# openfheorg/openfhe-boolean-circuit-evaluator

Measured on NVIDIA B200. Metric: bootstrapped gates/sec (STD128_OPT GINX), higher is better.
Workload: dtype u32

## Files before the change

openfhe-boolean-circuit-evaluator_b200/csrc/kernels.cu:

```cuda
#include "device.cuh"
#include <type_traits>
#include <cuda_runtime.h>
#include <cstdlib>

namespace bfhe {

constexpr int SOL_LAT_WIDE = 0x05, SOL_LAT_NARROW = 0x0a;

__device__ __forceinline__ u32 f_phys(u32 u) { return (u & ~31u) | ((u ^ (u >> 5)) & 31u); }
template <int E> struct Lay {
  static constexpr int C = E / 4;
  __device__ __forceinline__ static int swz(int tp) { return E == 32 ? (tp & 7) : ((tp >> 1) & 3); }
  __device__ __forceinline__ static int chunk_off(int tp, int c) { return E * tp + 4 * (c ^ swz(tp)); }
  __device__ __forceinline__ static int elem_off(int k, int lane) {
    if (E == 32) return 32 * k + 4 * ((lane >> 2) ^ (k & 7)) + (lane & 3);
    int j = lane & 15;
    return 16 * (2 * k + (lane >> 4)) + 4 * ((j >> 2) ^ (k & 3)) + (j & 3);
  }
};
template <int E> __device__ __forceinline__ void row_load(const u32 *buf, u32 (&x)[E], int lane) {
#pragma unroll
  for (int c = 0; c < E / 4; c++) {
    uint4 v = *reinterpret_cast<const uint4 *>(buf + Lay<E>::chunk_off(lane, c));
    x[4 * c] = v.x; x[4 * c + 1] = v.y; x[4 * c + 2] = v.z; x[4 * c + 3] = v.w;
// ... 78 lines not shown
        x[a] = RED ? lazy_reduce(S, Q) : S;
      }
    }
    if constexpr (!LAST) GsRun<E, 2 * T, OUTB, UNI, MAXLAST>::run(x, utw, utws, Q, tab, tabs, lane);
  }
};
__host__ __device__ constexpr int gs_out_bound(int E, int B0, int MAXLAST) {
  int B = B0;
  for (int T = 1; T < E; T *= 2) {
    const int NB = 2 * B;
    const bool last = 2 * T >= E;
    B = (last ? NB > MAXLAST : NB > 16) ? 2 : NB;
  }
  return B;
}

struct TwTabs {
  const u32 *fw, *fws, *iw, *iws;
};

template <int LOGN, bool PRE = false, int SOLW = 0, int SOLN = 0>
__device__ __forceinline__ void ntt_forward(u32 (&x)[(1 << LOGN) / 32], u32 *buf, const DevConst &P, const TwTabs &tt, int lane,
                                            const u32 *pre = nullptr) {
  constexpr int E = (1 << LOGN) / 32;
  const u32 Q = P.Q, Q2 = P.Q2;
  ct_pass<E, true, SOLW, PRE>(x, P.tw, P.tws, Q, Q2, nullptr, nullptr, 0, pre);
  if constexpr (LOGN & 1) {
    const bool up = lane & 16;
#pragma unroll
    for (int k = 0; k < E; k++) {
      u32 v = up ? mul_shoup(x[k], P.tw[16 + k], P.tws[16 + k], Q) : x[k];
      u32 o = __shfl_xor_sync(0xffffffffu, v, 16);
      x[k] = up ? (o - v + Q2) : (v + o);
    }
  }
  __syncwarp();
  col_store<E>(buf, x, lane);
  __syncwarp();
  row_load<E>(buf, x, lane);
  ct_pass<E, false, SOLN>(x, P.tw, P.tws, Q, Q2, tt.fw, tt.fws, lane);
}

template <int LOGN, int B0>
__device__ __forceinline__ void ntt_inverse(u32 (&x)[(1 << LOGN) / 32], u32 *buf, const DevConst &P, const TwTabs &tt, int lane) {
  constexpr int E = (1 << LOGN) / 32;
  const u32 Q = P.Q;
  constexpr int ML = (LOGN & 1) ? 8 : 16;
  GsRun<E, 1, B0, false, ML>::run(x, P.itw, P.itws, Q, tt.iw, tt.iws, lane);
  constexpr int B1 = gs_out_bound(E, B0, ML);
  __syncwarp();
  row_store<E>(buf, x, lane);
  __syncwarp();
  col_load<E>(buf, x, lane);
  if constexpr (LOGN & 1) {
    static_assert(B1 <= 8, "bound");
    const bool up = lane & 16;
    const u32 off = B1 * Q;
#pragma unroll
    for (int k = 0; k < E; k++) {
      u32 o = __shfl_xor_sync(0xffffffffu, x[k], 16);
      u32 D = o - x[k] + off;
      x[k] = up ? mul_shoup(D, P.itw[16 + k], P.itws[16 + k], Q) : (x[k] + o);
    }
    constexpr int B2 = 2 * B1;
    GsRun<E, 1, B2, true, 32>::run(x, P.itw, P.itws, Q);
  } else {
    GsRun<E, 1, B1, true, 32>::run(x, P.itw, P.itws, Q);
  }
#pragma unroll
  for (int k = 0; k < E; k++) x[k] = csub(lazy_reduce(x[k], Q), Q);
}

__device__ __forceinline__ u32 brev(u32 x, int bits) { return __brev(x) >> (32 - bits); }
template <int DG, int LOGBG> constexpr u32 digit_offset() {
  u32 off = 0;
  for (int l = 0; l < DG; l++) off += (1u << (LOGBG - 1)) << (LOGBG * l);
  return off;
}

template <int LOGN, int DG, int LOGBG, int G, bool AP> struct BrCfg {
  static constexpr int N = 1 << LOGN, E = N / 32, C = E / 4, ROWS = 2 * DG;
  static constexpr int W = 2 * G, THREADS = 32 * W;
  static constexpr int NPAD = AP ? 1024 : 512;
  static constexpr size_t dct_words = (size_t)G * ROWS * N;
  static constexpr bool LUT = (LOGBG == 7 && LOGN == 10);
  static constexpr size_t lut_words = LUT ? (size_t)32 << LOGBG : 0;
  static constexpr bool FOLD = LUT && !AP;
  static constexpr size_t smem_bytes = (dct_words + 4 * N + (AP ? 0 : 2 * N) + lut_words) * 4 + (size_t)G * NPAD * 2;
};

template <int LOGN, int DG, int LOGBG, int G, bool AP>
__global__ void __launch_bounds__(64 * G, 1)
blind_rotate_kernel(const __grid_constant__ DevConst P, const DevGate *__restrict__ gates, int count,
                    const u32 *__restrict__ bk, const u32 *__restrict__ g_twl, const u32 *__restrict__ g_psiM,
                    u32 *__restrict__ ext, u32 *__restrict__ acc_dbg) {
  using Cfg = BrCfg<LOGN, DG, LOGBG, G, AP>;
  constexpr int N = Cfg::N, E = Cfg::E, C = Cfg::C, ROWS = Cfg::ROWS, W = Cfg::W, NPAD = Cfg::NPAD;
  constexpr u32 DIGIT_OFF = digit_offset<DG, LOGBG>();
  constexpr bool FOLD = Cfg::FOLD;
  static_assert(!FOLD || (DIGIT_OFF >= (SOLINAS_Q + 1) / 2 && (u64)DIGIT_OFF + (SOLINAS_Q - 3) / 2 < (1ull << (LOGBG * DG))),
                "the digits do not cover the centred accumulator: the top digit cannot be folded into the key");
  constexpr int ND = FOLD ? DG - 1 : DG;
  extern __shared__ __align__(128) unsigned char smem_raw[];
  u32 *dct = reinterpret_cast<u32 *>(smem_raw);
  u32 *s_tw = dct + Cfg::dct_words;
  u32 *s_psiM = s_tw + 4 * N;
  u32 *s_lut = s_psiM + (AP ? 0 : 2 * N);
  u16 *s_idx = reinterpret_cast<u16 *>(s_lut + Cfg::lut_words);

  const int tid = threadIdx.x, lane = tid & 31, warp = tid >> 5;
  const int g = warp >> 1, c = warp & 1;
  if constexpr (Cfg::LUT) {
    for (int i = tid; i < (int)Cfg::lut_words; i += Cfg::THREADS) {
      const u32 d = (u32)i >> 5;
      s_lut[i] = (u32)(((u64)P.tw[1] * ((d + P.Q - (1u << (LOGBG - 1))) % P.Q)) % P.Q);
    }
  }
  const int gate0 = blockIdx.x * G;
  const int gcount = min(G, count - gate0);
  const u32 Q = P.Q, q = P.q, n = P.n;

  for (int i = tid; i < 4 * N; i += Cfg::THREADS) s_tw[i] = g_twl[i];
  if (!AP)
    for (int u = tid; u < N; u += Cfg::THREADS) s_psiM[f_phys((u32)u)] = (g_psiM[2 * u] + (P.Q - P.oneM)) % P.Q;
  const TwTabs tt{s_tw, s_tw + N, s_tw + 2 * N, s_tw + 3 * N};

  __shared__ u32 s_b[G];
  for (int gg = 0; gg < gcount; gg++) {
    const DevGate dg = gates[gate0 + gg];
    const u32 gate = dg.op & 0xff;
    for (u32 i = tid; i <= n; i += Cfg::THREADS) {
      u32 x = dg.in0[i];
      if (dg.op & OP_NEG0) x = (i == n) ? (q / 4 + q - x) % q : (q - x) % q;
      u32 v;
      if (gate == OP_BOOTSTRAP) {
        v = (i == n) ? (x + q / 4) % q : x;
      } else {
        u32 y = dg.in1[i];
        if (dg.op & OP_NEG1) y = (i == n) ? (q / 4 + q - y) % q : (q - y) % q;
        v = (gate == OP_XOR_FAST || gate == OP_XNOR_FAST) ? (2 * (x + q - y)) % q : (x + y) % q;
      }
      if (i == n) s_b[gg] = v;
      else {
        u32 aneg = (q - v) % q;
        if (!AP) s_idx[gg * NPAD + i] = (u16)(aneg * P.factor);
        else {
          u32 a = aneg;
          for (u32 k = 0; k < P.dR; k++, a /= P.baseR) s_idx[gg * NPAD + i * P.dR + k] = (u16)(a % P.baseR);
        }
      }
    }
  }
  __syncthreads();

  const bool gvalid = g < gcount;
  u32 acc[E];
#pragma unroll
  for (int k = 0; k < E; k++) acc[k] = 0;
  if (gvalid && c == 1) {
    const u32 gate = gates[gate0 + g].op & 0xff;
    const u32 q1 = P.gate_const[gate == OP_BOOTSTRAP ? OP_AND : gate], q2 = (q1 + q / 2) % q;
    const u32 b = s_b[g], Q8 = P.Q8, Q8n = Q - P.Q8;
#pragma unroll
    for (int k = 0; k < E; k++) {
      const u32 idx = lane + 32 * k;
      if (idx % P.factor == 0) {
        const u32 t = (b + q - idx / P.factor) % q;
        const bool in = (q1 < q2) ? (t >= q1 && t < q2) : !(t >= q2 && t < q1);
        acc[k] = in ? Q8n : Q8;
      }
    }
  }
  if (FOLD && gvalid) {
    u32 x[E];
#pragma unroll
    for (int k = 0; k < E; k++) x[k] = acc[k];
    u32 *abuf = dct + ((size_t)g * ROWS + 2 * (DG - 1) + c) * N;
    ntt_forward<LOGN>(x, abuf, P, tt, lane);
#pragma unroll
    for (int k = 0; k < E; k++) x[k] = mul_shoup(x[k], P.ninv, P.ninvs, Q);
    row_store<E>(abuf, x, lane);
  }

  const int nsteps = AP ? n * P.dR : n;
  bool pending = false;
  u32 *mybuf = dct + ((size_t)g * ROWS + c) * N;

  constexpr int GS = (W >= C) ? (W / C) : 1;
  const u32 eA = 2 * brev(lane, 5) + 1;
  constexpr bool KEY_HOIST = !AP;

#ifdef BFHE_PHASE_TIMING
  long long tpt[5] = {0, 0, 0, 0, 0}, tq0 = clock64(), tq1;
#define PT_T(i) do { tq1 = clock64(); tpt[i] += tq1 - tq0; tq0 = tq1; } while (0)
#else
#define PT_T(i)
#endif
  for (int step = 0; step < nsteps; step++) {
    uint4 kr[2][ROWS][2];
#define BFHE_GX_LOAD(qc)                                     \
  do {                                                                                                                 \
    const u32 *kb_ = bk + (size_t)step * (2 * ROWS * 2) * N + ((qc) * 32 + lane) * 4;                                  \
    _Pragma("unroll") for (int s = 0; s < 2; s++)                                                                      \
      _Pragma("unroll") for (int r = 0; r < ROWS; r++)                                                                 \
        _Pragma("unroll") for (int cc = 0; cc < 2; cc++)                                                               \
          kr[s][r][cc] = __ldg(reinterpret_cast<const uint4 *>(kb_ + (size_t)((s * ROWS + r) * 2 + cc) * N));           \
  } while (0)
    constexpr int JN = (G + GS - 1) / GS;
    auto ap_key = [&](int gg, int qc) -> const u32 * {
      const u32 a0 = gg < gcount ? s_idx[gg * NPAD + step] : 0u;
      const u32 i = step / P.dR, k = step % P.dR;
      return bk + (((size_t)i * (P.baseR - 1) + (a0 ? a0 - 1 : 0u)) * P.dR + k) * (ROWS * 2) * N + (qc * 32 + lane) * 4;
    };
#define BFHE_AP_LOAD(buf, kb)                                                                                          \
  do {                                                                                                                 \
    const u32 *kb_ = (kb);                                                                                             \
    _Pragma("unroll") for (int r = 0; r < ROWS; r++)                                                                   \
      _Pragma("unroll") for (int cc = 0; cc < 2; cc++)                                                                 \
        kr[buf][r][cc] = __ldg(reinterpret_cast<const uint4 *>(kb_ + (size_t)(r * 2 + cc) * N));                        \
  } while (0)

    bool active = gvalid;
    if (AP && gvalid) active = s_idx[g * NPAD + step] != 0;
    if (active) {
      if (pending) {
        u32 x[E];
        row_load<E>(mybuf, x, lane);
        ntt_inverse<LOGN, AP ? 8 : 4>(x, mybuf, P, tt, lane);
#pragma unroll
        for (int k = 0; k < E; k++) acc[k] = AP ? x[k] : csub(acc[k] + x[k], Q);
      }
      u32 dp[E];
#pragma unroll
      for (int k = 0; k < E; k++) dp[k] = ((acc[k] < (Q >> 1)) ? acc[k] : acc[k] - Q) + DIGIT_OFF;
#pragma unroll
      for (int l = 0; l < ND; l++) {
        u32 x[E], pre[Cfg::LUT ? E / 2 : 1];
#pragma unroll
        for (int k = 0; k < E; k++) {
          const u32 dgt = (dp[k] >> (LOGBG * l)) & ((1u << LOGBG) - 1);
          if (Cfg::LUT && k >= E / 2) { pre[Cfg::LUT ? k - E / 2 : 0] = s_lut[(dgt << 5) + lane]; x[k] = 0; }
          else x[k] = dgt + (Q - (1u << (LOGBG - 1)));
        }
        u32 *buf = dct + ((size_t)g * ROWS + c + 2 * l) * N;
        if (KEY_HOIST && l == ND - 1 && warp < C * GS) BFHE_GX_LOAD(warp % C);
        ntt_forward<LOGN, Cfg::LUT>(x, buf, P, tt, lane, pre);
        row_store<E>(buf, x, lane);
      }
    } else if (KEY_HOIST && warp < C * GS) {
      BFHE_GX_LOAD(warp % C);
    }
    pending = pending || active;
    PT_T(0);
    if (AP && warp < C * GS) {
      BFHE_AP_LOAD(0, ap_key(warp / C, warp % C));
      if (JN > 1) BFHE_AP_LOAD(1, ap_key(warp / C + GS, warp % C));
    }
    __syncthreads();
    PT_T(1);

    for (int item = warp; item < C * GS; item += W) {
      const int qc = item % C, gs0 = item / C;
      if (!AP && item != warp) BFHE_GX_LOAD(qc);
      u32 eB[4];
#pragma unroll
      for (int r = 0; r < 4; r++) eB[r] = 2 * ((brev(r, 2) << (LOGN - 2)) | (brev(qc, LOGN - 7) << 5));

      if (AP && item != warp) {
        BFHE_AP_LOAD(0, ap_key(gs0, qc));
        if (JN > 1) BFHE_AP_LOAD(1, ap_key(gs0 + GS, qc));
      }
#pragma unroll
      for (int j = 0; j < JN; j++) {
        const int gg = gs0 + j * GS;
        const bool ap_active = AP && gg < gcount && s_idx[(gg < gcount ? gg : 0) * NPAD + step] != 0;
        if (gg >= gcount || (AP && !ap_active)) {
          if (AP && j + 2 < JN) { if ((j & 1) == 0) BFHE_AP_LOAD(0, ap_key(gs0 + (j + 2) * GS, qc)); else BFHE_AP_LOAD(1, ap_key(gs0 + (j + 2) * GS, qc)); }
          continue;
        }
        u32 fp[4], fn[4];
        if (!AP) {
          const u32 m = s_idx[gg * NPAD + step];
#pragma unroll
          for (int r = 0; r < 4; r++) {
            const u32 u = ((m * (eA + eB[r])) >> 1) & (N - 1);
            fp[r] = s_psiM[f_phys(u)];
            fn[r] = s_psiM[f_phys((0u - u) & (N - 1))];
          }
        }
        u32 *gd = dct + (size_t)gg * ROWS * N + Lay<E>::chunk_off(lane, qc);
        uint4 dv[ROWS];
#pragma unroll
        for (int r = 0; r < ROWS; r++) dv[r] = *reinterpret_cast<const uint4 *>(gd + (size_t)r * N);
#pragma unroll
        for (int cc = 0; cc < 2; cc++) {
          u32 out[4];
#pragma unroll
          for (int sl = 0; sl < 4; sl++) {
            u64 sp = 0, sn = 0;
#pragma unroll
            for (int r = 0; r < ROWS; r++) {
              const u32 dval = sl == 0 ? dv[r].x : sl == 1 ? dv[r].y : sl == 2 ? dv[r].z : dv[r].w;
              const uint4 kp = kr[AP ? (j & 1) : 0][r][cc];
              sp += (u64)dval * (sl == 0 ? kp.x : sl == 1 ? kp.y : sl == 2 ? kp.z : kp.w);
              if (!AP) {
                const uint4 kn = kr[AP ? 0 : 1][r][cc];
                sn += (u64)dval * (sl == 0 ? kn.x : sl == 1 ? kn.y : sl == 2 ? kn.z : kn.w);
              }
            }
            const u32 pp = redc(sp, Q, P.qinv_neg);
            if (AP) out[sl] = pp;
            else {
              const u32 pn = redc(sn, Q, P.qinv_neg);
              out[sl] = redc((u64)pp * fp[sl] + (u64)pn * fn[sl], Q, P.qinv_neg);
            }
          }
          *reinterpret_cast<uint4 *>(gd + (size_t)cc * N) = make_uint4(out[0], out[1], out[2], out[3]);
          if constexpr (FOLD) {
            const uint4 a = dv[ROWS - 2 + cc];
            *reinterpret_cast<uint4 *>(gd + (size_t)(ROWS - 2 + cc) * N) =
                make_uint4(lazy_reduce(a.x + out[0], Q), lazy_reduce(a.y + out[1], Q), lazy_reduce(a.z + out[2], Q), lazy_reduce(a.w + out[3], Q));
          }
        }
        if (AP && j + 2 < JN) {
          if ((j & 1) == 0) BFHE_AP_LOAD(0, ap_key(gs0 + (j + 2) * GS, qc)); else BFHE_AP_LOAD(1, ap_key(gs0 + (j + 2) * GS, qc));
        }
      }
    }
    PT_T(2);
    __syncthreads();
    PT_T(3);
  }

  if (gvalid) {
    if (pending) {
      u32 x[E];
      row_load<E>(mybuf, x, lane);
      ntt_inverse<LOGN, AP ? 8 : 4>(x, mybuf, P, tt, lane);
#pragma unroll
      for (int k = 0; k < E; k++) acc[k] = AP ? x[k] : csub(acc[k] + x[k], Q);
    }
    const size_t gi = (size_t)gate0 + g;
    if (acc_dbg) {
#pragma unroll
      for (int k = 0; k < E; k++) acc_dbg[(gi * 2 + c) * N + lane + 32 * k] = acc[k];
    }
    u32 *e = ext + gi * (N + 4);
    const u64 qKS = P.qKS;
    if (c == 0) {
#pragma unroll
      for (int k = 0; k < E; k++) {
        const u32 j = lane + 32 * k;
        const u32 v = (j == 0) ? acc[k] : (acc[k] == 0 ? 0 : Q - acc[k]);
        const u32 pos = (j == 0) ? 0 : N - j;
        e[pos] = (qKS == Q) ? v : (u32)(((2 * (u64)v * qKS + Q) / (2 * (u64)Q)) % qKS);
      }
    } else if (lane == 0) {
      const u32 v = csub(acc[0] + P.Q8, Q);
      e[N] = (qKS == Q) ? v : (u32)(((2 * (u64)v * qKS + Q) / (2 * (u64)Q)) % qKS);
    }
#ifdef BFHE_PHASE_TIMING
    if (acc_dbg && lane == 0)
      for (int i = 0; i < 5; i++) acc_dbg[(gi * 2 + c) * N + 32 + i] = (u32)(tpt[i] / 1000);
#endif
  }
}



template <int T, int B> struct Gs8Stage {
  static constexpr bool RED = (2 * B > 16);
  static constexpr int OUTB = RED ? 2 : 2 * B;
  __device__ __forceinline__ static void run(u32 (&x)[8], const u32 (&w)[8], const u32 (&ws)[8], u32 Q) {
    static_assert(B <= 16, "bound");
#pragma unroll
    for (int i = 0; i < 4; i++) {
      const int gi = i / T, a = gi * 2 * T + (i % T), b = a + T, p = 4 / T + gi;
      const u32 S = x[a] + x[b], D = x[a] - x[b] + B * Q;
      x[b] = mul_shoup(D, w[p], ws[p], Q);
      x[a] = RED ? lazy_reduce(S, Q) : S;
    }
  }
};
template <int B0> __device__ __forceinline__ void ntt_inverse_quad8(u32 (&x)[8], u32 *buf, const DevConst &P, const u32 *nat, const u32 *nats, int T,
                                                                   int bar_id) {
  const u32 Q = P.Q;
  u32 w[8], ws[8];
  auto run3 = [&](auto BC) {
    constexpr int B = decltype(BC)::value;
    using S1 = Gs8Stage<1, B>; using S2 = Gs8Stage<2, S1::OUTB>; using S3 = Gs8Stage<4, S2::OUTB>;
    S1::run(x, w, ws, Q); S2::run(x, w, ws, Q); S3::run(x, w, ws, Q);
  };
  constexpr int B1 = Gs8Stage<4, Gs8Stage<2, Gs8Stage<1, B0>::OUTB>::OUTB>::OUTB;
  constexpr int B2 = Gs8Stage<4, Gs8Stage<2, Gs8Stage<1, B1>::OUTB>::OUTB>::OUTB;
  constexpr int B3 = Gs8Stage<4, Gs8Stage<2, Gs8Stage<1, B2>::OUTB>::OUTB>::OUTB;
  {
    const int tp = T >> 2, c0 = 2 * (T & 3), T3 = T >> 1, hb = T & 1;
    u32 *p0 = buf + Lay<32>::chunk_off(tp, c0), *p1 = buf + Lay<32>::chunk_off(tp, c0 + 1);
    const uint4 a0 = *reinterpret_cast<const uint4 *>(p0), a1 = *reinterpret_cast<const uint4 *>(p1);
    x[0] = a0.x; x[1] = a0.y; x[2] = a0.z; x[3] = a0.w; x[4] = a1.x; x[5] = a1.y; x[6] = a1.z; x[7] = a1.w;
    const uint4 t4 = *reinterpret_cast<const uint4 *>(nat + 512 + 256 * hb + 4 * T3), t4s = *reinterpret_cast<const uint4 *>(nats + 512 + 256 * hb + 4 * T3);
    const uint2 t2 = *reinterpret_cast<const uint2 *>(nat + 256 + 2 * T), t2s = *reinterpret_cast<const uint2 *>(nats + 256 + 2 * T);
    w[4] = t4.x; w[5] = t4.y; w[6] = t4.z; w[7] = t4.w; ws[4] = t4s.x; ws[5] = t4s.y; ws[6] = t4s.z; ws[7] = t4s.w;
    w[2] = t2.x; w[3] = t2.y; ws[2] = t2s.x; ws[3] = t2s.y;
    w[1] = nat[128 + T]; ws[1] = nats[128 + T];
    run3(std::integral_constant<int, B0>{});
    *reinterpret_cast<uint4 *>(p0) = make_uint4(x[0], x[1], x[2], x[3]);
    *reinterpret_cast<uint4 *>(p1) = make_uint4(x[4], x[5], x[6], x[7]);
  }
  bar_sync(bar_id, 128);
  {
    const int u = T >> 3, v = T & 7;
    const int b = 64 * u + 8 * (u & 3) + 4 * (v >> 2) + (v & 3);
    const uint4 t4 = *reinterpret_cast<const uint4 *>(nat + 64 + 4 * u), t4s = *reinterpret_cast<const uint4 *>(nats + 64 + 4 * u);
    const uint2 t2 = *reinterpret_cast<const uint2 *>(nat + 32 + 2 * u), t2s = *reinterpret_cast<const uint2 *>(nats + 32 + 2 * u);
    w[4] = t4.x; w[5] = t4.y; w[6] = t4.z; w[7] = t4.w; ws[4] = t4s.x; ws[5] = t4s.y; ws[6] = t4s.z; ws[7] = t4s.w;
    w[2] = t2.x; w[3] = t2.y; ws[2] = t2s.x; ws[3] = t2s.y;
    w[1] = nat[16 + u]; ws[1] = nats[16 + u];
#pragma unroll
    for (int r = 0; r < 8; r++) x[r] = buf[b ^ (32 * (r >> 2) + 8 * (r & 3) + 4 * (r >> 2))];
    run3(std::integral_constant<int, B1>{});
#pragma unroll
    for (int r = 0; r < 8; r++) buf[b ^ (32 * (r >> 2) + 8 * (r & 3) + 4 * (r >> 2))] = x[r];
  }
// ... 288 lines not shown
    } else if (lane == 0) {
      e[N] = modswitch(csub(acc[0] + P.Q8, Q));
    }
  }
#ifdef BFHE_PHASE_TIMING
  if (acc_dbg && lane == 0 && (QUAD ? (q4 == 0) : (warp < 2)))
    for (int i = 0; i < 5; i++) acc_dbg[(gi * 2 + (QUAD ? qc : warp)) * N + 32 + i] = (u32)(tph[i] / 1000);
#endif
}

template <int LOGN, int DG, int LOGBG, bool AP>
static int launch_lat_inst(const DevConst &P, const DevGate *d_gates, int count, const u32 *d_bk, const u32 *d_twl,
                           const u32 *d_psiM, u32 *d_ext, u32 *d_acc, cudaStream_t st, LaunchInfo *info) {
  using Cfg = LatCfg<LOGN, DG, LOGBG, AP>;
  auto kern = blind_rotate_lat_kernel<LOGN, DG, LOGBG, AP>;
  static bool attr_done[64];
  if (int rc = once_per_device(attr_done, [&] { return cudaFuncSetAttribute(kern, cudaFuncAttributeMaxDynamicSharedMemorySize, (int)Cfg::smem_bytes); }))
    return rc;
  if (count <= 0) return 0;
  if (info) { info->gates_per_cta = 1; info->ctas = count; info->smem_bytes = Cfg::smem_bytes; }
  kern<<<count, Cfg::THREADS, Cfg::smem_bytes, st>>>(P, d_gates, count, d_bk, d_twl, d_psiM, d_ext, d_acc);
  return (int)cudaGetLastError();
}

template <int LOGN, int DG, int LOGBG, int G, bool AP>
static int launch_br_inst(const DevConst &P, const DevGate *d_gates, int count, const u32 *d_bk, const u32 *d_twl,
                          const u32 *d_psiM, u32 *d_ext, u32 *d_acc, cudaStream_t st, LaunchInfo *info) {
  using Cfg = BrCfg<LOGN, DG, LOGBG, G, AP>;
  auto kern = blind_rotate_kernel<LOGN, DG, LOGBG, G, AP>;
  static bool attr_done[64];
  if (int rc = once_per_device(attr_done, [&] { return cudaFuncSetAttribute(kern, cudaFuncAttributeMaxDynamicSharedMemorySize, (int)Cfg::smem_bytes); }))
    return rc;
  if (count <= 0) return 0;
  const int ctas = (count + G - 1) / G;
  if (info) { info->gates_per_cta = G; info->ctas = ctas; info->smem_bytes = Cfg::smem_bytes; }
  kern<<<ctas, Cfg::THREADS, Cfg::smem_bytes, st>>>(P, d_gates, count, d_bk, d_twl, d_psiM, d_ext, d_acc);
  return (int)cudaGetLastError();
}

template <int LOGN, int DG, int LOGBG, bool AP>
static int launch_br_g(int G, const DevConst &P, const DevGate *d_gates, int count, const u32 *d_bk, const u32 *d_twl,
                       const u32 *d_psiM, u32 *d_ext, u32 *d_acc, cudaStream_t st, LaunchInfo *info) {
  switch (G) {
  case 1: return launch_br_inst<LOGN, DG, LOGBG, 1, AP>(P, d_gates, count, d_bk, d_twl, d_psiM, d_ext, d_acc, st, info);
  case 2: return launch_br_inst<LOGN, DG, LOGBG, 2, AP>(P, d_gates, count, d_bk, d_twl, d_psiM, d_ext, d_acc, st, info);
  default: return launch_br_inst<LOGN, DG, LOGBG, 4, AP>(P, d_gates, count, d_bk, d_twl, d_psiM, d_ext, d_acc, st, info);
  }
}

template <int LOGN, int DG, int LOGBG> static int br_attrs() {
  DevConst P{};
  int rc = 0;
  for (int G : {1, 2, 4}) {
    rc |= launch_br_g<LOGN, DG, LOGBG, false>(G, P, nullptr, 0, nullptr, nullptr, nullptr, nullptr, nullptr, 0, nullptr);
    rc |= launch_br_g<LOGN, DG, LOGBG, true>(G, P, nullptr, 0, nullptr, nullptr, nullptr, nullptr, nullptr, 0, nullptr);
  }
  rc |= launch_lat_inst<LOGN, DG, LOGBG, false>(P, nullptr, 0, nullptr, nullptr, nullptr, nullptr, nullptr, 0, nullptr);
  rc |= launch_lat_inst<LOGN, DG, LOGBG, true>(P, nullptr, 0, nullptr, nullptr, nullptr, nullptr, nullptr, 0, nullptr);
  return rc;
}
int blind_rotate_set_attrs() {
  int rc = br_attrs<10, 4, 7>();
  rc |= br_attrs<9, 3, 9>();
  rc |= v2_set_attrs();
  rc |= clx_set_attrs();
  return rc;
}

int launch_blind_rotate(const DevConst &P, int method_ap, const DevGate *d_gates, int count, const u32 *d_bk, const u32 *d_twl,
                        const u32 *d_psiM, u32 *d_ext, u32 *d_acc_dbg, int force_g, void *stream, LaunchInfo *info, const V2Bufs *v2) {
  if (count <= 0) return 0;
  cudaStream_t st = (cudaStream_t)stream;
  const bool have_cl2 = v2 && v2->d_bk4 && v2->d_tw2 && v2->d_F && v2_supported(P, method_ap);
  const bool have_clx = v2 && v2->d_bkx && v2->d_twx && (method_ap || v2->d_F) && clx_supported(P, method_ap);
  if (force_g == 128) return have_clx ? launch_blind_rotate_clx(P, method_ap, d_gates, count, *v2, d_ext, d_acc_dbg, stream, info) : (int)cudaErrorInvalidValue;
  if (force_g == 32) return have_cl2 ? launch_blind_rotate_cl2(P, d_gates, count, *v2, d_ext, d_acc_dbg, stream, info) : (int)cudaErrorInvalidValue;
  if (force_g != 0 && force_g != 1 && force_g != 2 && force_g != 4 && force_g != 8) return (int)cudaErrorInvalidValue;
  int dev = 0, sms = 148;
  cudaGetDevice(&dev);
  cudaDeviceGetAttribute(&sms, cudaDevAttrMultiProcessorCount, dev);
  if (force_g == 0 && have_clx && count <= clx_fast_gates()) return launch_blind_rotate_clx(P, method_ap, d_gates, count, *v2, d_ext, d_acc_dbg, stream, info);
  if (force_g == 0 && have_cl2 && count <= cl2_max_gates()) return launch_blind_rotate_cl2(P, d_gates, count, *v2, d_ext, d_acc_dbg, stream, info);
  const long lat_cost = (long)((count + sms - 1) / sms) * 222;
  const long thr_cost = (long)((count + 4 * sms - 1) / (4 * sms)) * 597;
  const bool lat = force_g == 8 || (force_g == 0 && lat_cost <= thr_cost);
  if (lat) {
    if (P.N == 1024 && P.dG == 4 && P.logBG == 7)
      return method_ap ? launch_lat_inst<10, 4, 7, true>(P, d_gates, count, d_bk, d_twl, d_psiM, d_ext, d_acc_dbg, st, info)
                       : launch_lat_inst<10, 4, 7, false>(P, d_gates, count, d_bk, d_twl, d_psiM, d_ext, d_acc_dbg, st, info);
    if (P.N == 512 && P.dG == 3 && P.logBG == 9)
      return method_ap ? launch_lat_inst<9, 3, 9, true>(P, d_gates, count, d_bk, d_twl, d_psiM, d_ext, d_acc_dbg, st, info)
                       : launch_lat_inst<9, 3, 9, false>(P, d_gates, count, d_bk, d_twl, d_psiM, d_ext, d_acc_dbg, st, info);
    return (int)cudaErrorInvalidValue;
  }
  int G = force_g > 0 ? force_g : 4;
  if (P.N == 1024 && P.dG == 4 && P.logBG == 7) {
    if (method_ap) return launch_br_g<10, 4, 7, true>(G, P, d_gates, count, d_bk, d_twl, d_psiM, d_ext, d_acc_dbg, st, info);
    static_assert(BrCfg<10, 4, 7, 4, false>::FOLD, "the GINX throughput kernel of this shape reads the folded key");
    if (!v2 || !v2->d_bkf) return (int)cudaErrorInvalidValue;
    return launch_br_g<10, 4, 7, false>(G, P, d_gates, count, v2->d_bkf, d_twl, d_psiM, d_ext, d_acc_dbg, st, info);
  }
  if (P.N == 512 && P.dG == 3 && P.logBG == 9) {
    return method_ap ? launch_br_g<9, 3, 9, true>(G, P, d_gates, count, d_bk, d_twl, d_psiM, d_ext, d_acc_dbg, st, info)
                     : launch_br_g<9, 3, 9, false>(G, P, d_gates, count, d_bk, d_twl, d_psiM, d_ext, d_acc_dbg, st, info);
  }
  return (int)cudaErrorInvalidValue;
}

__device__ __forceinline__ void peer_store(const PeerX &px, const u32 *out, int k, u32 v) {
  if (px.slabs == nullptr) return;
  const size_t off = (size_t)(out - px.local_base) + (size_t)k;
  for (u32 r = 0; r < px.world; r++)
    if (r != px.rank) px.slabs[r][off] = v;
}
__device__ __forceinline__ void st_release_sys(u32 *p, u32 v) { asm volatile("st.release.sys.global.u32 [%0], %1;" ::"l"(p), "r"(v) : "memory"); }
__device__ __forceinline__ u32 ld_acquire_sys(const u32 *p) {
  u32 v;
  asm volatile("ld.acquire.sys.global.u32 %0, [%1];" : "=r"(v) : "l"(p) : "memory");
  return v;
}
__device__ __forceinline__ void peer_publish(const PeerX &px, u32 total) {
  if (px.slabs == nullptr) return;
  __threadfence_system();
  __syncthreads();
  if (threadIdx.x == 0) {
    const u32 done = atomicAdd(px.counter, 1u) + 1u;
    if (done == total) {
      atomicExch(px.counter, 0u);
      __threadfence_system();
      const u32 v = *px.epoch * px.per_epoch + px.index + 1u;
      for (u32 r = 0; r < px.world; r++)
        if (r != px.rank) st_release_sys(px.flags[r] + px.rank, v);
    }
  }
}
__global__ void peer_epoch_bump_kernel(u32 *epoch) { *epoch += 1; }
__global__ void peer_wait_kernel(const u32 *flags, const u32 *epoch, u32 world, u32 rank, int index, u32 per_epoch, u32 *err, long long timeout_cycles) {
  const u32 r = threadIdx.x;
  if (r >= world || r == rank) return;
  const u32 target = *epoch * per_epoch + (u32)(index + 1);
  const long long t0 = clock64();
  while ((int)(ld_acquire_sys(flags + r) - target) < 0) {
    if (clock64() - t0 > timeout_cycles) { atomicExch(err, 1u + r); break; }
    __nanosleep(200);
  }
}
__global__ void peer_signal_kernel(const PeerX px) {
  const u32 r = threadIdx.x;
  if (r >= px.world || r == px.rank) return;
  __threadfence_system();
  st_release_sys(px.flags[r] + px.rank, *px.epoch * px.per_epoch + px.index + 1u);
}
int launch_peer_epoch_bump(u32 *epoch, void *stream) {
  peer_epoch_bump_kernel<<<1, 1, 0, (cudaStream_t)stream>>>(epoch);
  return (int)cudaGetLastError();
}
int launch_peer_wait(const u32 *local_flags, const u32 *epoch, u32 world, u32 rank, int index, u32 per_epoch, u32 *err, void *stream) {
  if (world > 32) return (int)cudaErrorInvalidValue;
  static const long long cycles = [] {
    const char *e = std::getenv("BFHE_EXCHANGE_TIMEOUT_S");
    const double sec = e && std::atof(e) > 0 ? std::atof(e) : 30.0;
    return (long long)(sec * 2.0e9);
  }();
  peer_wait_kernel<<<1, 32, 0, (cudaStream_t)stream>>>(local_flags, epoch, world, rank, index, per_epoch, err, cycles);
  return (int)cudaGetLastError();
}
int launch_peer_signal(const PeerX &px, void *stream) {
// ... 332 lines not shown
```

openfhe-boolean-circuit-evaluator_b200/host/circuit.cpp:

```cpp
#include "../csrc/engine.hpp"
#include "netlist.hpp"
#include <algorithm>
#include <chrono>
#include <cstdio>
#include <cstdlib>
#include <cstring>
#include <dlfcn.h>
#include <queue>

using namespace bfhe;

namespace {

struct Id128 { char b[128]; };
struct NcclApi {
  void *h = nullptr;
  int (*GetUniqueId)(void *) = nullptr;
  int (*CommInitRank)(void **, int, Id128, int) = nullptr;
  int (*AllGather)(const void *, void *, size_t, int, void *, cudaStream_t) = nullptr;
  int (*Broadcast)(const void *, void *, size_t, int, int, void *, cudaStream_t) = nullptr;
  int (*CommDestroy)(void *) = nullptr;
  const char *(*GetErrorString)(int) = nullptr;
};
NcclApi g_nccl;
bool load_nccl() {
  if (g_nccl.h) return true;
  void *h = dlopen("libnccl.so.2", RTLD_NOW | RTLD_GLOBAL);
  if (!h) h = dlopen("libnccl.so", RTLD_NOW | RTLD_GLOBAL);
  if (!h) { set_error(std::string("cannot load NCCL: ") + dlerror()); return false; }
  g_nccl.GetUniqueId = (decltype(g_nccl.GetUniqueId))dlsym(h, "ncclGetUniqueId");
  g_nccl.CommInitRank = (decltype(g_nccl.CommInitRank))dlsym(h, "ncclCommInitRank");
  g_nccl.AllGather = (decltype(g_nccl.AllGather))dlsym(h, "ncclAllGather");
  g_nccl.Broadcast = (decltype(g_nccl.Broadcast))dlsym(h, "ncclBroadcast");
  g_nccl.CommDestroy = (decltype(g_nccl.CommDestroy))dlsym(h, "ncclCommDestroy");
  g_nccl.GetErrorString = (decltype(g_nccl.GetErrorString))dlsym(h, "ncclGetErrorString");
  if (!g_nccl.GetUniqueId || !g_nccl.CommInitRank || !g_nccl.AllGather || !g_nccl.Broadcast || !g_nccl.CommDestroy) {
    set_error("NCCL symbols missing");
    return false;
  }
  g_nccl.h = h;
  return true;
}
constexpr int NCCL_UINT32 = 3, NCCL_FLOAT32 = 7;

struct NotOp { uint32_t in_row, out_row, copy; };
struct Level {
  std::vector<bfhe_gate> gates;
  uint32_t first_row = 0;
  std::vector<NotOp> nots;
  bool sharded = true;
};
struct FormCosts {
  double cl4 = 1.05, cl2 = 1.55, lat = 2.36, thr = 6.1, exchange = exchange_default();
  bool measured = false;
  static double exchange_default() { const char *m = std::getenv("BFHE_EXCHANGE"); return m && std::strcmp(m, "nccl") == 0 ? 0.05 : 0.015; }
};
inline bool is_single(GateKind k) {
  return k == GateKind::AND || k == GateKind::OR || k == GateKind::NAND || k == GateKind::NOR || k == GateKind::XOR_FAST || k == GateKind::XNOR_FAST;
}
inline bool is_boot(GateKind k) { return is_single(k) || k == GateKind::XOR; }
inline uint32_t op_of(GateKind k) {
  switch (k) {
  case GateKind::AND: return BFHE_AND;
  case GateKind::OR: return BFHE_OR;
  case GateKind::NAND: return BFHE_NAND;
  case GateKind::NOR: return BFHE_NOR;
  case GateKind::XOR_FAST: return BFHE_XOR_FAST;
  default: return BFHE_XNOR_FAST;
  }
}

}

struct bfhe_circuit {
  bfhe_ctx *ctx = nullptr;
  Netlist nl;
  Netlist nl_file;
  bool loaded = false;
  bool plaintext = false, encrypted = false, verify = false;
  bool planned_verify = false;
  int rank = 0, world = 1;
  void *comm = nullptr;

  bool planned = false;
  std::vector<uint32_t> topo;
  std::vector<uint32_t> wire_row;
  std::vector<uint8_t> wire_neg;
  std::vector<uint32_t> wire_level;
  std::vector<Level> levels;
  std::vector<uint32_t> level_rpr;
  uint32_t total_rows = 0, fresh_base = 0, n_in = 0;
  std::vector<uint32_t> in_wire_of_bit;
  std::vector<uint32_t> out_wire;
  uint32_t n_bootstraps = 0, max_width = 0, asap_levels = 0;
  uint32_t wave_cap = 0;
  int wave_cap_req = -1;
  int shard_min_req = -1;
  FormCosts costs;
  uint32_t n_dff = 0, state_base = 0, dff_tmp_base = 0, dff_fresh_base = 0;
  std::vector<uint32_t> dff_gate;
  std::vector<NotOp> dff_ops;
  std::vector<uint8_t> plain_state;
  bool state_init_pending = true;
  uint64_t clocks = 0;

  uint32_t *slab = nullptr;
  DevGate *d_desc = nullptr;
  std::vector<size_t> desc_off;
  std::vector<uint32_t> my_count;
  const u32 **d_not_in = nullptr;
  u32 **d_not_out = nullptr;
  std::vector<size_t> not_off;
  u32 *d_ext = nullptr;
  size_t ext_cap = 0;
  bool dev_ready = false;
  cudaGraphExec_t graph = nullptr;
  bool use_graph = true;
  bool peer_ok = false;
  std::vector<void *> peer_slab_map, peer_flag_map;
  u32 **d_peer_slabs = nullptr, **d_peer_flags = nullptr;
  u32 *x_flags = nullptr, *x_counter = nullptr, *x_epoch = nullptr, *x_err = nullptr;
  uint32_t x_per_epoch = 1;
  std::vector<int> shard_index;

  std::vector<uint8_t> in_bits_set, plain_wire;
  bool has_input = false, done = false;
  double device_ms = 0, host_ms = 0;
  uint64_t verify_mismatches = 0, verify_checked = 0;
};

static void free_device(bfhe_circuit *c) {
  if (c->ctx && c->ctx->device >= 0) {
    cudaSetDevice(c->ctx->device);
    cudaStreamSynchronize(c->ctx->stream);
    if (c->graph) cudaGraphExecDestroy(c->graph);
    for (void *m : c->peer_slab_map) if (m) cudaIpcCloseMemHandle(m);
// ... 1093 lines not shown
```

Measured before the change: 97800.

## Keep blind-rotate accumulator in NTT domain in shared memory across steps

The throughput blind-rotate kernel now keeps the accumulator transformed (A_hat rows in shared memory) for every configuration. The external product adds into A_hat directly, and each step recovers the coefficient form with one inverse NTT of A_hat. Before, it inverted the product and added it to a register accumulator. This removes the pending-accumulate bookkeeping and register-resident acc across steps. For the non-fold cases it costs two extra shared-memory rows per gate and an extra NTT at setup. The host cost-model constants for the throughput path are lowered to match.

Result: faster. 101,900 (median of 6 runs) (+4.2%).

```diff
diff --git a/openfhe-boolean-circuit-evaluator_b200/csrc/kernels.cu b/openfhe-boolean-circuit-evaluator_b200/csrc/kernels.cu
--- a/openfhe-boolean-circuit-evaluator_b200/csrc/kernels.cu
+++ b/openfhe-boolean-circuit-evaluator_b200/csrc/kernels.cu
@@ -184,11 +184,14 @@
   static constexpr int N = 1 << LOGN, E = N / 32, C = E / 4, ROWS = 2 * DG;
   static constexpr int W = 2 * G, THREADS = 32 * W;
   static constexpr int NPAD = AP ? 1024 : 512;
-  static constexpr size_t dct_words = (size_t)G * ROWS * N;
   static constexpr bool LUT = (LOGBG == 7 && LOGN == 10);
   static constexpr size_t lut_words = LUT ? (size_t)32 << LOGBG : 0;
   static constexpr bool FOLD = LUT && !AP;
+  static constexpr int DROWS = (FOLD || AP) ? ROWS : ROWS + 2;
+  static constexpr int AROW = AP ? 0 : DROWS - 2;
+  static constexpr size_t dct_words = (size_t)G * DROWS * N;
   static constexpr size_t smem_bytes = (dct_words + 4 * N + (AP ? 0 : 2 * N) + lut_words) * 4 + (size_t)G * NPAD * 2;
+  static_assert(smem_bytes <= 227 * 1024, "more dynamic shared memory than a block may have");
 };
 
 template <int LOGN, int DG, int LOGBG, int G, bool AP>
@@ -203,6 +206,9 @@
   static_assert(!FOLD || (DIGIT_OFF >= (SOLINAS_Q + 1) / 2 && (u64)DIGIT_OFF + (SOLINAS_Q - 3) / 2 < (1ull << (LOGBG * DG))),
                 "the digits do not cover the centred accumulator: the top digit cannot be folded into the key");
   constexpr int ND = FOLD ? DG - 1 : DG;
+  constexpr int DROWS = Cfg::DROWS, AROW = Cfg::AROW;
+  static_assert(AP || AROW == 2 * ND, "GINX: the A_hat rows follow the digit rows");
+  constexpr int AB = AP ? 8 : 2;
   extern __shared__ __align__(128) unsigned char smem_raw[];
   u32 *dct = reinterpret_cast<u32 *>(smem_raw);
   u32 *s_tw = dct + Cfg::dct_words;
@@ -256,37 +262,33 @@
   __syncthreads();
 
   const bool gvalid = g < gcount;
-  u32 acc[E];
-#pragma unroll
-  for (int k = 0; k < E; k++) acc[k] = 0;
-  if (gvalid && c == 1) {
-    const u32 gate = gates[gate0 + g].op & 0xff;
-    const u32 q1 = P.gate_const[gate == OP_BOOTSTRAP ? OP_AND : gate], q2 = (q1 + q / 2) % q;
-    const u32 b = s_b[g], Q8 = P.Q8, Q8n = Q - P.Q8;
-#pragma unroll
-    for (int k = 0; k < E; k++) {
-      const u32 idx = lane + 32 * k;
-      if (idx % P.factor == 0) {
-        const u32 t = (b + q - idx / P.factor) % q;
-        const bool in = (q1 < q2) ? (t >= q1 && t < q2) : !(t >= q2 && t < q1);
-        acc[k] = in ? Q8n : Q8;
-      }
-    }
-  }
-  if (FOLD && gvalid) {
-    u32 x[E];
-#pragma unroll
-    for (int k = 0; k < E; k++) x[k] = acc[k];
-    u32 *abuf = dct + ((size_t)g * ROWS + 2 * (DG - 1) + c) * N;
-    ntt_forward<LOGN>(x, abuf, P, tt, lane);
-#pragma unroll
-    for (int k = 0; k < E; k++) x[k] = mul_shoup(x[k], P.ninv, P.ninvs, Q);
-    row_store<E>(abuf, x, lane);
+  u32 *ahat = dct + ((size_t)g * DROWS + AROW + c) * N;
+  u32 *dbuf = dct + ((size_t)g * DROWS + c) * N;
+  if (gvalid) {
+    u32 acc[E];
+#pragma unroll
+    for (int k = 0; k < E; k++) acc[k] = 0;
+    if (c == 1) {
+      const u32 gate = gates[gate0 + g].op & 0xff;
+      const u32 q1 = P.gate_const[gate == OP_BOOTSTRAP ? OP_AND : gate], q2 = (q1 + q / 2) % q;
+      const u32 b = s_b[g], Q8 = P.Q8, Q8n = Q - P.Q8;
+#pragma unroll
+      for (int k = 0; k < E; k++) {
+        const u32 idx = lane + 32 * k;
+        if (idx % P.factor == 0) {
+          const u32 t = (b + q - idx / P.factor) % q;
+          const bool in = (q1 < q2) ? (t >= q1 && t < q2) : !(t >= q2 && t < q1);
+          acc[k] = in ? Q8n : Q8;
+        }
+      }
+    }
+    ntt_forward<LOGN>(acc, ahat, P, tt, lane);
+#pragma unroll
+    for (int k = 0; k < E; k++) acc[k] = mul_shoup(acc[k], P.ninv, P.ninvs, Q);
+    row_store<E>(ahat, acc, lane);
   }
 
   const int nsteps = AP ? n * P.dR : n;
-  bool pending = false;
-  u32 *mybuf = dct + ((size_t)g * ROWS + c) * N;
 
   constexpr int GS = (W >= C) ? (W / C) : 1;
   const u32 eA = 2 * brev(lane, 5) + 1;
@@ -325,16 +327,11 @@
     bool active = gvalid;
     if (AP && gvalid) active = s_idx[g * NPAD + step] != 0;
     if (active) {
-      if (pending) {
-        u32 x[E];
-        row_load<E>(mybuf, x, lane);
-        ntt_inverse<LOGN, AP ? 8 : 4>(x, mybuf, P, tt, lane);
-#pragma unroll
-        for (int k = 0; k < E; k++) acc[k] = AP ? x[k] : csub(acc[k] + x[k], Q);
-      }
       u32 dp[E];
-#pragma unroll
-      for (int k = 0; k < E; k++) dp[k] = ((acc[k] < (Q >> 1)) ? acc[k] : acc[k] - Q) + DIGIT_OFF;
+      row_load<E>(ahat, dp, lane);
+      ntt_inverse<LOGN, AB>(dp, dbuf, P, tt, lane);
+#pragma unroll
+      for (int k = 0; k < E; k++) dp[k] = ((dp[k] < (Q >> 1)) ? dp[k] : dp[k] - Q) + DIGIT_OFF;
 #pragma unroll
       for (int l = 0; l < ND; l++) {
         u32 x[E], pre[Cfg::LUT ? E / 2 : 1];
@@ -344,7 +341,7 @@
           if (Cfg::LUT && k >= E / 2) { pre[Cfg::LUT ? k - E / 2 : 0] = s_lut[(dgt << 5) + lane]; x[k] = 0; }
           else x[k] = dgt + (Q - (1u << (LOGBG - 1)));
         }
-        u32 *buf = dct + ((size_t)g * ROWS + c + 2 * l) * N;
+        u32 *buf = dct + ((size_t)g * DROWS + c + 2 * l) * N;
         if (KEY_HOIST && l == ND - 1 && warp < C * GS) BFHE_GX_LOAD(warp % C);
         ntt_forward<LOGN, Cfg::LUT>(x, buf, P, tt, lane, pre);
         row_store<E>(buf, x, lane);
@@ -352,7 +349,6 @@
     } else if (KEY_HOIST && warp < C * GS) {
       BFHE_GX_LOAD(warp % C);
     }
-    pending = pending || active;
     PT_T(0);
     if (AP && warp < C * GS) {
       BFHE_AP_LOAD(0, ap_key(warp / C, warp % C));
@@ -390,10 +386,11 @@
             fn[r] = s_psiM[f_phys((0u - u) & (N - 1))];
           }
         }
-        u32 *gd = dct + (size_t)gg * ROWS * N + Lay<E>::chunk_off(lane, qc);
-        uint4 dv[ROWS];
-#pragma unroll
-        for (int r = 0; r < ROWS; r++) dv[r] = *reinterpret_cast<const uint4 *>(gd + (size_t)r * N);
+        u32 *gd = dct + (size_t)gg * DROWS * N + Lay<E>::chunk_off(lane, qc);
+        constexpr int NLD = AP ? ROWS : DROWS;
+        uint4 dv[NLD];
+#pragma unroll
+        for (int r = 0; r < NLD; r++) dv[r] = *reinterpret_cast<const uint4 *>(gd + (size_t)r * N);
 #pragma unroll
         for (int cc = 0; cc < 2; cc++) {
           u32 out[4];
@@ -417,10 +414,11 @@
               out[sl] = redc((u64)pp * fp[sl] + (u64)pn * fn[sl], Q, P.qinv_neg);
             }
           }
-          *reinterpret_cast<uint4 *>(gd + (size_t)cc * N) = make_uint4(out[0], out[1], out[2], out[3]);
-          if constexpr (FOLD) {
-            const uint4 a = dv[ROWS - 2 + cc];
-            *reinterpret_cast<uint4 *>(gd + (size_t)(ROWS - 2 + cc) * N) =
+          u32 *ga = gd + (size_t)(AROW + cc) * N;
+          if constexpr (AP) *reinterpret_cast<uint4 *>(ga) = make_uint4(out[0], out[1], out[2], out[3]);
+          else {
+            const uint4 a = dv[AROW + cc];
+            *reinterpret_cast<uint4 *>(ga) =
                 make_uint4(lazy_reduce(a.x + out[0], Q), lazy_reduce(a.y + out[1], Q), lazy_reduce(a.z + out[2], Q), lazy_reduce(a.w + out[3], Q));
           }
         }
@@ -435,13 +433,9 @@
   }
 
   if (gvalid) {
-    if (pending) {
-      u32 x[E];
-      row_load<E>(mybuf, x, lane);
-      ntt_inverse<LOGN, AP ? 8 : 4>(x, mybuf, P, tt, lane);
-#pragma unroll
-      for (int k = 0; k < E; k++) acc[k] = AP ? x[k] : csub(acc[k] + x[k], Q);
-    }
+    u32 acc[E];
+    row_load<E>(ahat, acc, lane);
+    ntt_inverse<LOGN, AB>(acc, dbuf, P, tt, lane);
     const size_t gi = (size_t)gate0 + g;
     if (acc_dbg) {
 #pragma unroll
@@ -896,7 +890,7 @@
   if (force_g == 0 && have_clx && count <= clx_fast_gates()) return launch_blind_rotate_clx(P, method_ap, d_gates, count, *v2, d_ext, d_acc_dbg, stream, info);
   if (force_g == 0 && have_cl2 && count <= cl2_max_gates()) return launch_blind_rotate_cl2(P, d_gates, count, *v2, d_ext, d_acc_dbg, stream, info);
   const long lat_cost = (long)((count + sms - 1) / sms) * 222;
-  const long thr_cost = (long)((count + 4 * sms - 1) / (4 * sms)) * 597;
+  const long thr_cost = (long)((count + 4 * sms - 1) / (4 * sms)) * 568;
   const bool lat = force_g == 8 || (force_g == 0 && lat_cost <= thr_cost);
   if (lat) {
     if (P.N == 1024 && P.dG == 4 && P.logBG == 7)
diff --git a/openfhe-boolean-circuit-evaluator_b200/host/circuit.cpp b/openfhe-boolean-circuit-evaluator_b200/host/circuit.cpp
--- a/openfhe-boolean-circuit-evaluator_b200/host/circuit.cpp
+++ b/openfhe-boolean-circuit-evaluator_b200/host/circuit.cpp
@@ -51,7 +51,7 @@
   bool sharded = true;
 };
 struct FormCosts {
-  double cl4 = 1.05, cl2 = 1.55, lat = 2.36, thr = 6.1, exchange = exchange_default();
+  double cl4 = 1.05, cl2 = 1.55, lat = 2.36, thr = 5.85, exchange = exchange_default();
   bool measured = false;
   static double exchange_default() { const char *m = std::getenv("BFHE_EXCHANGE"); return m && std::strcmp(m, "nccl") == 0 ? 0.05 : 0.015; }
 };
```
